# gau-nernst/centernet-lightning

Hardware: AMD Instinct MI355X
Metric: images/sec @512x512 ResNet34 CenterNet forward + gather_detection2d (higher is better)
Workload: dtype f32; 1 GPU; BASELINE C1: ResNet34 + simple neck, 32 img/GPU x 512x512, heads 80+4 (w256), k=100, nms 3; global_batch=32, per_gpu_batch=32, parallelism=batch-shard x1

## Files before the change

### centernet-lightning_amd/centernet_lightning_amd/_lib.py

```python
import ctypes
import os
from ctypes import (POINTER, Structure, c_char_p, c_double, c_float, c_int32, c_int64, c_size_t, c_uint32, c_void_p)

_LIB_NAME = "libcenternet_gfx950.so"
_LIB_PATH = os.path.join(os.path.dirname(os.path.abspath(__file__)), "lib", _LIB_NAME)

CNL_RELU = 1 << 0
CNL_SIGMOID = 1 << 1
CNL_UPSAMPLE_IN = 1 << 2
CNL_UPSAMPLE_OUT_ADD = 1 << 3
CNL_RELU6 = 1 << 4
CNL_W_SPLIT = 1 << 5

CNL_ALGO_AUTO, CNL_ALGO_F2, CNL_ALGO_F32, CNL_ALGO_LATENCY, CNL_ALGO_F43, CNL_ALGO_FORCE = 0, 1, 2, 4, 5, 100
CNL_WINO_F32, CNL_WINO_F16X2 = 2, 5

CNL_E_BAD_ARG, CNL_E_UNSUPPORTED, CNL_E_WORKSPACE, CNL_E_HIP = -1, -2, -3, -4
ABI_VERSION = 13


class ConvParams(Structure):
    _fields_ = [("x", c_void_p), ("w", c_void_p), ("bias", c_void_p), ("residual", c_void_p), ("y", c_void_p),
                ("N", c_int32), ("H_in", c_int32), ("W_in", c_int32), ("Cin", c_int32), ("Cout", c_int32),
                ("KH", c_int32), ("KW", c_int32), ("stride", c_int32), ("pad", c_int32),
                ("ldx", c_int32), ("ldy", c_int32), ("ldr", c_int32), ("flags", c_uint32),
                ("x_absmax", c_void_p), ("y_absmax", c_void_p), ("w_absmax", c_void_p), ("algo", c_uint32),
                ("splitk", c_int32), ("splitk_scratch", c_void_p), ("splitk_scratch_bytes", c_size_t),
                ("fuse_w", c_void_p), ("fuse_part", c_void_p), ("w_up", c_void_p)]


class DeconvParams(Structure):
    _fields_ = [("x", c_void_p), ("w", c_void_p), ("bias", c_void_p), ("residual", c_void_p), ("y", c_void_p),
                ("N", c_int32), ("H_in", c_int32), ("W_in", c_int32), ("Cin", c_int32), ("Cout", c_int32), ("K", c_int32),
                ("ldx", c_int32), ("ldy", c_int32), ("ldr", c_int32), ("flags", c_uint32)]

# ... 180 lines not shown
```

### centernet-lightning_amd/centernet_lightning_amd/engine.py

```python
import bisect
import ctypes
import threading
from collections import OrderedDict
from dataclasses import dataclass

import torch

from . import _lib
from ._lib import (CNL_ALGO_AUTO, CNL_ALGO_F2, CNL_ALGO_F32, CNL_ALGO_F43, CNL_ALGO_FORCE, CNL_ALGO_LATENCY, CNL_RELU, CNL_RELU6, CNL_SIGMOID, CNL_UPSAMPLE_IN, CNL_UPSAMPLE_OUT_ADD, CNL_W_SPLIT,
                   CNL_WINO_F16X2, ConvParams, DeconvParams)

BN_EPS_DEFAULT = 1e-5


@dataclass(frozen=True)
class KernelOptions:
    algo: str = "auto"
    winograd: bool = True
    up2: bool = True
    absmax_handover: bool = True
    stem_fused_pool: bool = True
    presplit_weights: bool = True
    fuse_small_out: bool = True
    reuse_buffers: bool = True
    split_small: bool = False
    latency: bool = False
    up_rows: bool = True
    f43: bool = False
    check_range: bool = False

    @property
    def algo_id(self):
        try:
            return {"auto": CNL_ALGO_AUTO, "f2": CNL_ALGO_F2, "f32": CNL_ALGO_F32}[self.algo]
        except KeyError:
            raise ValueError(f"KernelOptions.algo must be 'auto', 'f2' or 'f32', got {self.algo!r}") from None


def fold_conv_bn(conv_w, conv_b, bn=None):
    w = conv_w.detach().to(torch.float32)
    cout = w.shape[0]
    b = conv_b.detach().to(torch.float32) if conv_b is not None else torch.zeros(cout, device=w.device)
    if bn is not None:
        scale = bn.weight.detach().float() / torch.sqrt(bn.running_var.detach().float() + bn.eps)
        w = w * scale.view(-1, 1, 1, 1)
        b = (b - bn.running_mean.detach().float()) * scale + bn.bias.detach().float()
# ... 53 lines not shown
            stream = ctypes.c_void_p(torch.cuda.current_stream(self.w.device).cuda_stream)
            _lib.check(lib.cnl_up2_pack_weights_f32(self.w.data_ptr(), self._up2.data_ptr(), self.cin, self.cout, stream), "cnl_up2_pack_weights_f32")
            self.up2_wmax = self._up2.abs().max().reshape(1).contiguous()
    return self._up2


def _layer_up_rows(self):
    if getattr(self, "_up_rows", None) is None:
        lib = _lib.load()
        n = lib.cnl_winograd_up_weight_floats(self.cin, self.cout) if (self.w.is_cuda and self.kh == 3 and self.kw == 3 and self.stride == 1) else 0
        if not n:
            self._up_rows = False
        else:
            with torch.cuda.device(self.w.device):
                buf = torch.empty((n,), device=self.w.device, dtype=torch.float32)
                stream = ctypes.c_void_p(torch.cuda.current_stream(self.w.device).cuda_stream)
                _lib.check(lib.cnl_winograd_transform_weights_up_f32(self.w.data_ptr(), buf.data_ptr(), self.cin, self.cout, stream),
                           "cnl_winograd_transform_weights_up_f32")
                torch.cuda.current_stream(self.w.device).synchronize()
            self._up_rows = buf
    return self._up_rows if self._up_rows is not False else None


_Layer.up_rows = _layer_up_rows
_Layer.split_w = _layer_split_w
_Layer.wants_up2 = _layer_wants_up2
_Layer.up2 = _layer_up2


class _Bottleneck:

    def __init__(self, c1, c2, c3, down, li):
        self.c1, self.c2, self.c3, self.down, self.li = c1, c2, c3, down, li
        self.cat = None
        if down is not None:
            self.cat = _Layer(torch.cat([c3.w, down.w], dim=3).contiguous(), (c3.b + down.b).contiguous())
            self.cat.k1 = c3.cin


class _SepLayer:

    def __init__(self, mod, device):
        w = mod.dw.weight.detach().to(device=device, dtype=torch.float32)
        bn = mod.dw_bn
        scale = (bn.weight.detach().float() / torch.sqrt(bn.running_var.detach().float() + bn.eps)).to(device)
        self.dw_w = (w[:, 0] * scale.view(-1, 1, 1)).permute(1, 2, 0).contiguous()
        self.dw_b = (bn.bias.detach().float().to(device) - bn.running_mean.detach().float().to(device) * scale).contiguous()
# ... 499 lines not shown
            elif self.options.f43 and self.algo in (CNL_ALGO_AUTO, CNL_ALGO_F2):
                p.algo = CNL_ALGO_F43
        rowwino = (fn is self.lib.cnl_conv3x3_winograd_f32 and self.algo != CNL_ALGO_F32
                   and self.lib.cnl_conv3x3_winograd_variant(ctypes.byref(p)) in (9, 10, 11))
        if rowwino and self.options.up_rows and (flags & CNL_UPSAMPLE_IN) and residual is None:
            wu = layer.up_rows()
            if wu is not None:
                p.w_up = wu.data_ptr()
        if (self.options.up2 and (flags & CNL_UPSAMPLE_IN) and not (flags & ~(CNL_RELU | CNL_UPSAMPLE_IN)) and residual is None
                and layer.wants_up2() and not rowwino):
            p.w = layer.up2().data_ptr()
            p.w_absmax = layer.up2_wmax.data_ptr()
            p.algo = self.algo
            fn = self.lib.cnl_conv3x3_up2_nhwc_f32
            what = what.replace(" [winograd]", "") + " [sub-pixel phases]"
        if fn is self.lib.cnl_conv2d_nhwc_f32 and self.options.presplit_weights and self.algo != CNL_ALGO_F32:
            ws = layer.split_w()
            if ws is not None:
                p.w = ws.data_ptr()
                p.flags |= CNL_W_SPLIT
        self.launches.append(_Launch(fn, p, what, flops, keep=(x, y, residual, layer)))
        return p, ho.value, wo.value

    def _bottlenecks(self, Wt, cur, ch, cw, cc, feats):
        N = self.N
        pw_ok = self.algo in (CNL_ALGO_AUTO, CNL_ALGO_F2) and self.options.absmax_handover and _POINTWISE_AB != "generic_auto"
        for j, blk in enumerate(Wt.blocks):
            c1, c2, c3, down, li = blk.c1, blk.c2, blk.c3, blk.down, blk.li
            bi = j - next(i for i, b in enumerate(Wt.blocks) if b.li == li)
            name = f"layer{li + 1}.{bi}"
            t1 = self._buf(N, ch, cw, c1.cout)
            self._conv1x1(c1, cur, ch, cw, cc, t1, CNL_RELU, pw_ok, what=f"{name}.conv1")
            oh, ow = (ch + 2 - 3) // c2.stride + 1, (cw + 2 - 3) // c2.stride + 1
            t2 = self._buf(N, oh, ow, c2.cout)
            self._conv(c2, t1, ch, cw, c1.cout, t2, c2.cout, CNL_RELU, what=f"{name}.conv2")
            out = self._buf(N, oh, ow, c3.cout)
            if down is not None and pw_ok and _POINTWISE_AB in (None, "pointwise_all"):
                self._pointwise(blk.cat, t2, oh, ow, c2.cout, out, CNL_RELU, x2=(cur, ch, cw, cc, down.stride), what=f"{name}.conv3+downsample")
            else:
                idn = cur
                if down is not None:
                    idn = self._buf(N, oh, ow, down.cout)
                    self._conv1x1(down, cur, ch, cw, cc, idn, 0, pw_ok, what=f"{name}.downsample")
                self._conv1x1(c3, t2, oh, ow, c2.cout, out, CNL_RELU, pw_ok, residual=idn, what=f"{name}.conv3")
            cur, ch, cw, cc = out, oh, ow, c3.cout
            feats[li] = (cur, ch, cw, cc)
# ... 141 lines not shown
        self._wt_stem_packed = Wt.stem_packed
        if H % 32 or W % 32:
            raise ValueError(f"input H, W must be divisible by 32 (got {H}x{W}); docs/implementation.md:52 of the reference")
        h2, w2 = (H + 6 - 7) // 2 + 1, (W + 6 - 7) // 2 + 1
        h4, w4 = (h2 + 2 - 3) // 2 + 1, (w2 + 2 - 3) // 2 + 1
        cur = self._buf(N, h4, w4, 64)
        need_s1 = (Wt.neck_kind != "SimpleNeck" and len(Wt.fuse) >= 4) or not self.options.stem_fused_pool or self.algo == CNL_ALGO_F32
        s1 = self._buf(N, h2, w2, 64) if need_s1 else None
        self.stem_out = s1 if need_s1 else cur
        self.stem_fused_pool = not need_s1
        self.backbone_in = cur
        self.stem_absmax = None
        self.launches.append(_Launch("stem", None, "stem7x7+bn+relu" + ("" if need_s1 else "+maxpool3x3s2"), 2 * N * h2 * w2 * 64 * 147,
                                     keep=(self.stem_out,)))
        if need_s1:
            self.launches.append(_Launch("maxpool", (s1, cur, N, h2, w2, 64), "maxpool3x3s2", keep=(s1, cur)))
        ch, cw, cc = h4, w4, 64
        feats = {}
        if Wt.bottleneck:
            cur, ch, cw, cc = self._bottlenecks(Wt, cur, ch, cw, cc, feats)
        for bi, (c1, c2, down, li) in enumerate(() if Wt.bottleneck else Wt.blocks):
            oh, ow = (ch + 2 - 3) // c1.stride + 1, (cw + 2 - 3) // c1.stride + 1
            t = self._buf(N, oh, ow, c1.cout)
            self._conv(c1, cur, ch, cw, cc, t, c1.cout, CNL_RELU, what=f"layer{li + 1}.{bi}.conv1")
            if down is not None:
                idn = self._buf(N, oh, ow, down.cout)
                self._conv(down, cur, ch, cw, cc, idn, down.cout, 0, what=f"layer{li + 1}.{bi}.downsample")
            else:
                idn = cur
            out = self._buf(N, oh, ow, c2.cout)
            self._conv(c2, t, oh, ow, c1.cout, out, c2.cout, CNL_RELU, residual=idn, ldr=c2.cout, what=f"layer{li + 1}.{bi}.conv2")
            cur, ch, cw, cc = out, oh, ow, c2.cout
            feats[li] = (cur, ch, cw, cc)
        self.features = [(s1, h2, w2, 64)] + [feats[i] for i in range(4)]

        bil = 1 if Wt.upsample_type == "bilinear" else 0
        if Wt.neck_kind == "SimpleNeck":
            x, xh, xw, xc = self.features[-1]
            up = 0
            for i, (layer, dec) in enumerate(zip(Wt.neck_layers, Wt.neck_ups)):
                if up and isinstance(layer, (_SepLayer, _DeformLayer)):
                    x, xh, xw, up = self._upsample(x, xh, xw, xc, xc, 0, f"neck.upsample.{i - 1} (nearest)"), 2 * xh, 2 * xw, 0
                y = self._buf(N, xh * (2 if up else 1), xw * (2 if up else 1), layer.cout)
                oh, ow = self._block(layer, x, xh, xw, xc, y, layer.cout, f"neck.layers.{i}", up)
                x, xh, xw, xc, up = y, oh, ow, layer.cout, 0
                if dec is not None:
                    x, xh, xw = self._deconv(dec, x, xh, xw, xc, f"neck.upsamples.{i} (conv_transpose)"), 2 * xh, 2 * xw
                elif bil:
                    x, xh, xw = self._upsample(x, xh, xw, xc, xc, 1, f"neck.upsample.{i} (bilinear)"), 2 * xh, 2 * xw
                else:
                    up = CNL_UPSAMPLE_IN
# ... 337 lines not shown
```

### centernet-lightning_amd/csrc/conv_args.h

```cpp
#pragma once
#include "cnl_device.h"

namespace cnl_conv {
using namespace cnl_dev;


struct ConvArgs {
    const float* x;
    const float* w;
    const float* bias;
    const float* res;
    float* y;
    int N, Hin, Win, Cin, Cout;
    int KH, KW, stride, pad, pad_x;
    int sub_dy, sub_dx;
    int ldx, ldy, ldr;
    int HL, WL;
    int Ho, Wo, M;
    int CC, KT, K;
    unsigned x_bytes, w_bytes, y_bytes, r_bytes;
    unsigned flags;
    int tiles_n, tiles;
    unsigned mg_hw, sh_hw, mg_w, sh_w;
    long long* trace;
    const float* xmax;
    const float* wmax;
    unsigned* ymax;
    unsigned algo;
    const float* wscale;
    const float* wsplit = nullptr;
    int ksplit = 0, kt_per = 0;
    float* part = nullptr;
    unsigned part_bytes = 0;
};

constexpr unsigned CNL_I_SUBPIXEL = 1u << 16;

template <int WM, int WN, int TM, int TN>
struct Cfg {
    static constexpr int NW = WM * WN;
    static constexpr int THREADS = NW * 64;
    static constexpr int BM = WM * TM * 32;
    static constexpr int BN = WN * TN * 32;
    static constexpr int A_INSTR = BM / (NW * 8);
    static constexpr int B_INSTR = BN / (NW * 8);
    static constexpr int STAGE_BYTES = (BM + BN) * 128;
    static constexpr int LDS_BYTES = 2 * STAGE_BYTES;
    static_assert(NW == 4, "kernel is declared __launch_bounds__(256, 2)");
    static_assert(BM % (NW * 8) == 0 && BN % (NW * 8) == 0, "tile rows must split evenly over waves");
};


__device__ __forceinline__ f32x4 buf_load4(const float* base, unsigned bytes, unsigned voffset, unsigned soffset) {
    const auto rsrc = __builtin_amdgcn_make_buffer_rsrc((void*)base, 0, (int)bytes, 0x00020000);
    return __builtin_bit_cast(f32x4, __builtin_amdgcn_raw_buffer_load_b128(rsrc, voffset, soffset, 0));
}
// ... 16 lines not shown
```

### centernet-lightning_amd/csrc/conv_f16x2.hip

```cpp
#include "conv_args.h"
#include <cstdlib>

namespace cnl_conv {



template <int WM, int WN, int TM, int TN, int KS, bool SUB, bool SPLIT = false, bool PREB = false>
__global__ __launch_bounds__(256, 2) void conv_f16x2_kernel(const ConvArgs a) {
    using C = Cfg<WM, WN, TM, TN>;
    constexpr bool PRE = SUB || PREB;
    extern __shared__ __attribute__((aligned(16))) char smem[];
    float* sInv = reinterpret_cast<float*>(smem + C::LDS_BYTES);
    float* sScl = sInv + C::BM;
    int* sImg = reinterpret_cast<int*>(sScl + C::BM);
    unsigned* sPix = reinterpret_cast<unsigned*>(sImg + C::BM);

    const int lane = threadIdx.x & 63;
    const int wave = __builtin_amdgcn_readfirstlane(threadIdx.x >> 6);
    const int wm = wave / WN, wn = wave % WN;
    const int hi = lane >> 5;

    unsigned tile = cnl::xcd_remap(blockIdx.x, (unsigned)a.tiles);
    int slice = 0;
    if constexpr (SPLIT) { slice = (int)(tile % (unsigned)a.ksplit); tile /= (unsigned)a.ksplit; }
    const int kt0 = SPLIT ? slice * a.kt_per : 0;
    const int KTs = SPLIT ? min(a.kt_per, a.KT - kt0) : a.KT;
    const int n_tile = tile % a.tiles_n;
    const int m_tile = tile / a.tiles_n;
    const int m0 = m_tile * C::BM;
    const int n0 = n_tile * C::BN;

    const int lrow = lane >> 3;
    const int pslot = lane & 7;
    unsigned a_mask[C::A_INSTR], a_base[C::A_INSTR];
#pragma unroll
    for (int j = 0; j < C::A_INSTR; ++j) {
        const int r = (j * C::NW + wave) * 8 + lrow;
        const int m = m0 + r;
        const int q = (pslot ^ ((r >> 1) & 7)) * 4;
        const unsigned n = fast_div((unsigned)m, a.mg_hw, a.sh_hw);
        const unsigned rem = (unsigned)m - n * (unsigned)(a.Ho * a.Wo);
        const unsigned oy = fast_div(rem, a.mg_w, a.sh_w);
        const unsigned ox = rem - oy * (unsigned)a.Wo;
        const int iy0 = (int)oy * a.stride - a.pad;
        const int ix0 = (int)ox * a.stride - a.pad_x;
        unsigned mask = 0, xb = 0;
#pragma unroll
        for (int kx = 0; kx < KS; ++kx) xb |= ((unsigned)(ix0 + kx) < (unsigned)a.WL) ? (1u << kx) : 0u;
#pragma unroll
// ... 3 lines not shown
        a_base[j] = (unsigned)(((pix + iy0 * a.Win + ix0) * a.ldx + q) * 4);
    }
    unsigned b_off[C::B_INSTR];
#pragma unroll
    for (int j = 0; j < C::B_INSTR; ++j) {
        const int r = (j * C::NW + wave) * 8 + lrow;
        const int q = (pslot ^ ((r >> 1) & 7)) * 4;
        b_off[j] = (unsigned)(((n0 + r) * a.K + q) * 4);
    }
    unsigned a_voff[C::A_INSTR];
#define C5_TAP(tap_, ky_, kx_)                                                                                    \
    do {                                                                                                          \
        const unsigned bit_ = 1u << (tap_);                                                                       \
        const unsigned delta_ = (unsigned)((((ky_) * a.Win + (kx_)) * a.ldx) * 4);                                \
        _Pragma("unroll") for (int j = 0; j < C::A_INSTR; ++j) a_voff[j] = (a_mask[j] & bit_) ? a_base[j] + delta_ : OOB; \
    } while (0)
#define C5_ISSUE(stage_, c0_, kbase_)                                                                             \
    do {                                                                                                          \
        char* sA_ = smem + (stage_) * C::STAGE_BYTES;                                                             \
        char* sB_ = sA_ + C::BM * 128;                                                                            \
        _Pragma("unroll") for (int j = 0; j < C::A_INSTR; ++j)                                                    \
            dma16(a.x, a.x_bytes, sA_ + (j * C::NW + wave) * 1024, a_voff[j], (unsigned)((c0_) * 4));             \
        _Pragma("unroll") for (int j = 0; j < C::B_INSTR; ++j)                                                    \
            dma16(PREB ? a.wsplit : a.w, a.w_bytes, sB_ + (j * C::NW + wave) * 1024, b_off[j], (unsigned)((kbase_) * 4)); \
    } while (0)
    int tap = 0, ky = 0, kx = 0, cc = 0;
#define C5_ADVANCE()                                    \
    do {                                                \
        if (++cc == a.CC) {                             \
            cc = 0;                                     \
            ++tap;                                      \
            if (++kx == KS) { kx = 0; ++ky; }           \
            C5_TAP(tap, ky, kx);                        \
        }                                               \
    } while (0)
    if constexpr (SPLIT) {
        tap = kt0 / a.CC; cc = kt0 - tap * a.CC; ky = tap / KS; kx = tap - ky * KS;
    }
    C5_TAP(tap, ky, kx);
    C5_ISSUE(0, cc * 32, kt0 * 32);

    const float Sw = PRE ? *a.wscale : pow2_scale(*a.wmax);
    for (int r = threadIdx.x; r < C::BM; r += C::THREADS) {
        const int m = m0 + r;
        const unsigned n = fast_div((unsigned)m, a.mg_hw, a.sh_hw);
        const bool ok = m < a.M;
        const float S = ok ? pow2_scale(a.xmax[n * AMS]) : 1.f;
        sScl[r] = S;
        sInv[r] = 1.f / (S * Sw);
        sImg[r] = ok ? (int)n : -1;
        if constexpr (SUB) {
            const unsigned rem = (unsigned)m - n * (unsigned)(a.Ho * a.Wo);
            const unsigned oy = fast_div(rem, a.mg_w, a.sh_w);
            const unsigned ox = rem - oy * (unsigned)a.Wo;
            sPix[r] = (n * 2u * (unsigned)a.Ho + 2u * oy + (unsigned)a.sub_dy) * (2u * (unsigned)a.Wo) + 2u * ox + (unsigned)a.sub_dx;
        }
    }

    f32x16 acc[TM][TN];
#pragma unroll
    for (int i = 0; i < TM; ++i)
#pragma unroll
        for (int j = 0; j < TN; ++j) acc[i][j] = mfma_zero();

    const int swz = (lane >> 1) & 7;
// ... 68 lines not shown
#undef C5_READ
#undef C5_SPLIT
#undef C5_MFMA

    if constexpr (SPLIT) {
#pragma unroll
        for (int j = 0; j < TN; ++j) {
            const int col = n0 + (wn * TN + j) * 32 + (lane & 31);
#pragma unroll
            for (int i = 0; i < TM; ++i) {
                const int rl = (wm * TM + i) * 32 + 4 * hi;
                const int mb = m0 + rl;
#pragma unroll
                for (int r = 0; r < 16; ++r) {
                    const int ro = (r & 3) + 8 * (r >> 2);
                    const bool ok = col < a.Cout && mb + ro < a.M;
                    buf_store(acc[i][j][r] * sInv[rl + ro], a.part, a.part_bytes,
                              ok ? (unsigned)((((long long)slice * a.M + mb + ro) * a.Cout + col) * 4) : OOB, 0u);
                }
            }
        }
        return;
    }
    const float lo = (a.flags & (CNL_RELU | CNL_RELU6)) ? 0.f : -__builtin_inff();
    const float hi6 = (a.flags & CNL_RELU6) ? 6.f : __builtin_inff();
    const bool sigm = a.flags & CNL_SIGMOID;
    const int img0 = sImg[0];
    float omax = 0.f, omax1 = 0.f;
#pragma unroll
    for (int j = 0; j < TN; ++j) {
        const int col = n0 + (wn * TN + j) * 32 + (lane & 31);
        const bool col_ok = col < a.Cout;
        const float bv = col_ok ? a.bias[col] : 0.f;
#pragma unroll
        for (int i = 0; i < TM; ++i) {
            const int rl = (wm * TM + i) * 32 + 4 * hi;
            const int mb = m0 + rl;
            const unsigned y_voff = (unsigned)((mb * a.ldy + col) * 4);
            const unsigned r_voff = (unsigned)((mb * a.ldr + col) * 4);
            float v[16];
            bool ok[16];
#pragma unroll
            for (int r = 0; r < 16; ++r) {
                const int ro = (r & 3) + 8 * (r >> 2);
                ok[r] = col_ok && mb + ro < a.M;
                v[r] = acc[i][j][r] * sInv[rl + ro] + bv;
            }
            if (!SUB && a.res) {
                float rv[16];
#pragma unroll
                for (int r = 0; r < 16; ++r)
                    rv[r] = buf_load(a.res, a.r_bytes, ok[r] ? r_voff : OOB, (unsigned)(((r & 3) + 8 * (r >> 2)) * a.ldr * 4));
#pragma unroll
                for (int r = 0; r < 16; ++r) v[r] += rv[r];
            }
#pragma unroll
            for (int r = 0; r < 16; ++r) v[r] = fminf(fmaxf(v[r], lo), hi6);
            if (sigm) {
#pragma unroll
                for (int r = 0; r < 16; ++r) v[r] = cnl::fast_sigmoid(v[r]);
            }
            if constexpr (SUB) {
#pragma unroll
                for (int r = 0; r < 16; ++r)
                    buf_store(v[r], a.y, a.y_bytes, ok[r] ? (sPix[rl + (r & 3) + 8 * (r >> 2)] * (unsigned)a.ldy + (unsigned)col) * 4u : OOB, 0u);
            } else {
#pragma unroll
                for (int r = 0; r < 16; ++r)
                    buf_store(v[r], a.y, a.y_bytes, ok[r] ? y_voff : OOB, (unsigned)(((r & 3) + 8 * (r >> 2)) * a.ldy * 4));
            }
            if (a.ymax) {
#pragma unroll
                for (int r = 0; r < 16; ++r) {
                    const float av = ok[r] ? fabsf(v[r]) : 0.f;
                    const int img = sImg[rl + (r & 3) + 8 * (r >> 2)];
                    if (img == img0) omax = fmaxf(omax, av);
                    else if (img == img0 + 1) omax1 = fmaxf(omax1, av);
                    else if (av > 0.f) cnl::report_max(a.ymax + img * AMS, av);
                }
            }
        }
    }
    if (a.ymax) {
#pragma unroll
        for (int o = 32; o > 0; o >>= 1) {
            omax = fmaxf(omax, __shfl_xor(omax, o, 64));
            omax1 = fmaxf(omax1, __shfl_xor(omax1, o, 64));
        }
        if (lane == 0) cnl::report_max(a.ymax + img0 * AMS, omax);
        if (lane == 0) cnl::report_max(a.ymax + (img0 + 1) * AMS, omax1);
    }
}

__global__ __launch_bounds__(256) void splitk_reduce_kernel(const ConvArgs a) {
    const int C4 = (a.Cout + 3) / 4;
    const long total = (long)a.M * C4;
    const long t = (long)blockIdx.x * 256 + threadIdx.x;
    float omax = 0.f;
    int img = -1;
    if (t < total) {
        const int m = (int)(t / C4), col = (int)(t - (long)m * C4) * 4;
        img = (int)fast_div((unsigned)m, a.mg_hw, a.sh_hw);
        const bool vec = col + 4 <= a.Cout && (a.Cout & 3) == 0;
        float v[4] = {0.f, 0.f, 0.f, 0.f};
        const long sstride = (long)a.M * a.Cout;
        const float* p0 = a.part + (long)m * a.Cout + col;
        if (vec) {
            for (int s0 = 0; s0 < a.ksplit; s0 += 8) {
                f32x4 q[8];
#pragma unroll
                for (int j = 0; j < 8; ++j)
                    q[j] = s0 + j < a.ksplit ? *reinterpret_cast<const f32x4*>(p0 + (s0 + j) * sstride) : f32x4{0.f, 0.f, 0.f, 0.f};
#pragma unroll
// ... 31 lines not shown
            atomicMax(a.ymax + img * AMS, __float_as_uint(omax));
        }
    }
}

template <int KS>
static int launch_split5(const ConvArgs& in, hipStream_t stream) {
    using C = Cfg<2, 2, 1, 2>;
    ConvArgs a = in;
    const int tiles_m = (a.M + C::BM - 1) / C::BM;
    a.tiles_n = (a.Cout + C::BN - 1) / C::BN;
    a.tiles = tiles_m * a.tiles_n * a.ksplit;
    static cnl::DeviceOnce once;
    int rc = cnl::kernel_setup(once, reinterpret_cast<const void*>(&conv_f16x2_kernel<2, 2, 1, 2, KS, false, true>), 160 * 1024);
    if (rc != CNL_OK) return rc;
    hipLaunchKernelGGL((conv_f16x2_kernel<2, 2, 1, 2, KS, false, true>), dim3(a.tiles), dim3(C::THREADS), C::LDS_BYTES + C::BM * 16, stream, a);
    rc = cnl::check_launch("conv_f16x2_kernel (split)");
    if (rc != CNL_OK) return rc;
    const long total = (long)a.M * ((a.Cout + 3) / 4);
    hipLaunchKernelGGL(splitk_reduce_kernel, dim3((unsigned)((total + 255) / 256)), dim3(256), 0, stream, a);
    return cnl::check_launch("splitk_reduce_kernel");
}

template <int WM, int WN, int TM, int TN, int KS, bool SUB, bool PREB = false>
static int launch_one5(const ConvArgs& a, hipStream_t stream) {
    using C = Cfg<WM, WN, TM, TN>;
    static cnl::DeviceOnce once;
    const int rc = cnl::kernel_setup(once, reinterpret_cast<const void*>(&conv_f16x2_kernel<WM, WN, TM, TN, KS, SUB, false, PREB>), 160 * 1024);
    if (rc != CNL_OK) return rc;
    hipLaunchKernelGGL((conv_f16x2_kernel<WM, WN, TM, TN, KS, SUB, false, PREB>), dim3(a.tiles), dim3(C::THREADS), C::LDS_BYTES + C::BM * 16, stream, a);
    return cnl::check_launch("conv_f16x2_kernel");
}

template <int WM, int WN, int TM, int TN>
static int launch_cfg5(const ConvArgs& in, hipStream_t stream) {
    using C = Cfg<WM, WN, TM, TN>;
    ConvArgs a = in;
    const int tiles_m = (a.M + C::BM - 1) / C::BM;
    a.tiles_n = (a.Cout + C::BN - 1) / C::BN;
    a.tiles = tiles_m * a.tiles_n;
    if (a.flags & CNL_I_SUBPIXEL) return launch_one5<WM, WN, TM, TN, 2, true>(a, stream);
    if (a.wsplit) return a.KH == 3 ? launch_one5<WM, WN, TM, TN, 3, false, true>(a, stream) : launch_one5<WM, WN, TM, TN, 1, false, true>(a, stream);
    return a.KH == 3 ? launch_one5<WM, WN, TM, TN, 3, false>(a, stream) : launch_one5<WM, WN, TM, TN, 1, false>(a, stream);
}

bool f16x2_eligible(const ConvArgs& a) {
    const long long min_out_1x1 = a.algo == CNL_ALGO_FORCE + 5 ? 0 : (1ll << 20);
    if (a.algo == CNL_ALGO_F32 || !a.xmax || (a.flags & (CNL_UPSAMPLE_IN | CNL_UPSAMPLE_OUT_ADD))) return false;
    if (a.flags & CNL_I_SUBPIXEL) return a.KH == 2 && a.KW == 2 && !a.res && a.wscale;
    return (a.wmax || (a.wsplit && a.ksplit <= 1)) && a.KH == a.KW && (a.KH == 1 || a.KH == 3) && a.pad == a.pad_x &&
           (a.KH == 3 || a.ksplit > 1 || (long long)a.Ho * a.Wo * a.Cout >= min_out_1x1);
}

int f16x2_launch(const ConvArgs& a, hipStream_t s) {
    if (a.ksplit > 1 && !(a.flags & CNL_I_SUBPIXEL)) return a.KH == 3 ? launch_split5<3>(a, s) : launch_split5<1>(a, s);
    if (a.Cout <= 32) return launch_cfg5<4, 1, 2, 1>(a, s);
    if (a.Cout <= 64) return launch_cfg5<4, 1, 2, 2>(a, s);
    if (a.Cout <= 96) return launch_cfg5<4, 1, 1, 3>(a, s);
    const long long tiles128 = (((long long)a.M + 127) / 128) * ((a.Cout + 127) / 128);
    if (tiles128 < 512) return launch_cfg5<2, 2, 1, 2>(a, s);
    return launch_cfg5<4, 1, 1, 4>(a, s);
}

}
```

### centernet-lightning_amd/csrc/conv_mfma.hip

```cpp
#include "conv_args.h"
#include <cstdlib>

namespace cnl_conv {

__device__ __forceinline__ f32x16 mfma32(float a, float b, f32x16 c) {
    return __builtin_amdgcn_mfma_f32_32x32x2f32(a, b, c, 0, 0, 0);
}
__device__ __forceinline__ f32x16 mfma_zero() {
    const f32x16 z = {0.f, 0.f, 0.f, 0.f, 0.f, 0.f, 0.f, 0.f, 0.f, 0.f, 0.f, 0.f, 0.f, 0.f, 0.f, 0.f};
    return __builtin_amdgcn_mfma_f32_32x32x2f32(0.f, 0.f, z, 0, 0, 0);
}
template <bool CHECK, bool RES>
__device__ __forceinline__ void store_tile(const f32x16& acc, float bv, float lo, float hi6, bool sigm, const ConvArgs& a, unsigned y_voff,
                                           unsigned r_voff, int m_base, bool col_ok) {
    float v[16];
    if constexpr (RES) {
        float rv[16];
#pragma unroll
        for (int r = 0; r < 16; ++r) {
            const int ro = (r & 3) + 8 * (r >> 2);
            const bool ok = !CHECK || (col_ok && m_base + ro < a.M);
            rv[r] = buf_load(a.res, a.r_bytes, ok ? r_voff : OOB, (unsigned)(ro * a.ldr * 4));
        }
#pragma unroll
// ... 429 lines not shown
static int finish_and_launch(ConvArgs& a, bool out4x, const char* who, hipStream_t s) {
    CNL_REQUIRE(a.Ho > 0 && a.Wo > 0, CNL_E_BAD_ARG, "%s: empty output", who);
    const long long M = (long long)a.N * a.Ho * a.Wo;
    CNL_REQUIRE(M < (1ll << 31) - 512, CNL_E_UNSUPPORTED, "%s: N*Ho*Wo too large", who);
    a.M = (int)M;
    a.CC = a.Cin / 32; a.KT = a.KH * a.KW * a.CC; a.K = a.KH * a.KW * a.Cin;
    const unsigned long long lim = 0xFFFFFF00ull;
    const unsigned long long xb = (((unsigned long long)a.N * a.Hin * a.Win - 1) * a.ldx + a.Cin) * 4ull;
    const unsigned long long wb = (unsigned long long)a.Cout * a.K * 4ull;
    const unsigned long long Mo = out4x ? 4ull * M : (unsigned long long)M;
    const unsigned long long yb = ((Mo - 1) * a.ldy + a.Cout) * 4ull;
    const unsigned long long rb = a.res ? ((Mo - 1) * a.ldr + a.Cout) * 4ull : 0ull;
    CNL_REQUIRE(xb < lim && yb + 512ull * a.ldy * 4 < lim && rb + 512ull * a.ldr * 4 < lim, CNL_E_UNSUPPORTED,
                "%s: a tensor spans >= 4 GiB (x %llu, y %llu bytes); split the batch", who, xb, yb);
    CNL_REQUIRE(wb + (unsigned long long)256 * a.K * 4ull < lim, CNL_E_UNSUPPORTED, "%s: weight too large", who);
    a.x_bytes = (unsigned)xb; a.w_bytes = (unsigned)wb; a.y_bytes = (unsigned)yb; a.r_bytes = (unsigned)rb;
    a.tiles_n = a.tiles = 0;
    magic_u31((unsigned)(a.Ho * a.Wo), &a.mg_hw, &a.sh_hw);
    magic_u31((unsigned)a.Wo, &a.mg_w, &a.sh_w);
    a.trace = nullptr;
#ifdef CNL_TRACE
    if (const char* e = getenv("CNL_TRACE_PTR")) a.trace = (long long*)strtoull(e, nullptr, 0);
#endif
    if (f16x2_eligible(a)) {
        if (a.ksplit > 1) {
            const int per = (a.KT + a.ksplit - 1) / a.ksplit;
            const unsigned long long pb = (unsigned long long)a.ksplit * (unsigned long long)M * a.Cout * 4ull;
            if (per >= 2 && !out4x && !(a.flags & CNL_UPSAMPLE_IN) && pb < lim) {
                a.kt_per = per;
                a.ksplit = (a.KT + per - 1) / per;
                a.part_bytes = (unsigned)((unsigned long long)a.ksplit * (unsigned long long)M * a.Cout * 4ull);
            } else {
                a.ksplit = 0;
            }
        }
        return f16x2_launch(a, s);
    }
    a.ksplit = 0;
    if (a.Cout <= 32) return launch_cfg<4, 1, 2, 1>(a, s);
    if (a.Cout <= 64) return launch_cfg<4, 1, 2, 2>(a, s);
    if (a.Cout <= 96) return launch_cfg<4, 1, 1, 3>(a, s);
    const long long tiles128 = ((M + 127) / 128) * ((a.Cout + 127) / 128);
    if (tiles128 < 512) return launch_cfg<2, 2, 1, 2>(a, s);
    return launch_cfg<2, 2, 2, 2>(a, s);
}

// ... 39 lines not shown
                "cnl_conv2d_nhwc_f32: Cin=%d is not a multiple of 32 (use cnl_stem_conv7x7_f32 for the RGB stem)", p->Cin);
    CNL_REQUIRE(p->ldx >= p->Cin && p->ldy >= p->Cout && p->ldx % 4 == 0, CNL_E_BAD_ARG,
                "cnl_conv2d_nhwc_f32: pixel strides ldx=%d ldy=%d too small / misaligned", p->ldx, p->ldy);
    CNL_REQUIRE(((uintptr_t)p->x & 15) == 0 && ((uintptr_t)p->w & 15) == 0, CNL_E_BAD_ARG,
                "cnl_conv2d_nhwc_f32: x and w must be 16-byte aligned");
    const bool up_out = p->flags & CNL_UPSAMPLE_OUT_ADD;
    CNL_REQUIRE(!up_out || p->residual, CNL_E_BAD_ARG, "cnl_conv2d_nhwc_f32: CNL_UPSAMPLE_OUT_ADD needs a residual");
    CNL_REQUIRE(!up_out || !(p->flags & CNL_SIGMOID), CNL_E_UNSUPPORTED, "cnl_conv2d_nhwc_f32: sigmoid with UPSAMPLE_OUT_ADD");
    CNL_REQUIRE(!p->residual || p->ldr >= p->Cout, CNL_E_BAD_ARG, "cnl_conv2d_nhwc_f32: ldr=%d < Cout", p->ldr);

    ConvArgs a;
    a.x = p->x; a.w = p->w; a.bias = p->bias; a.res = p->residual; a.y = p->y;
    a.N = p->N; a.Hin = p->H_in; a.Win = p->W_in; a.Cin = p->Cin; a.Cout = p->Cout;
    a.KH = p->KH; a.KW = p->KW; a.stride = p->stride; a.pad = a.pad_x = p->pad;
    a.sub_dy = a.sub_dx = 0;
    a.ldx = p->ldx; a.ldy = p->ldy; a.ldr = p->ldr;
    a.flags = p->flags;
    a.xmax = p->x_absmax; a.wmax = p->w_absmax; a.ymax = reinterpret_cast<unsigned*>(p->y_absmax); a.wscale = nullptr; a.algo = p->algo;
    if (p->flags & CNL_W_SPLIT) {
        CNL_REQUIRE(p->KH == p->KW && (p->KH == 1 || p->KH == 3), CNL_E_BAD_ARG, "cnl_conv2d_nhwc_f32: CNL_W_SPLIT with a %d x %d kernel", p->KH, p->KW);
        const size_t total = (size_t)p->Cout * p->KH * p->KW * p->Cin;
        a.wsplit = p->w + total;
        a.wscale = p->w + 2 * total;
    }
    const int up = (p->flags & CNL_UPSAMPLE_IN) ? 2 : 1;
    a.HL = p->H_in * up; a.WL = p->W_in * up;
    a.Ho = (a.HL + 2 * p->pad - p->KH) / p->stride + 1;
    a.Wo = (a.WL + 2 * p->pad - p->KW) / p->stride + 1;
    if (p->splitk > 1) {
        CNL_REQUIRE(p->splitk <= 256, CNL_E_BAD_ARG, "cnl_conv2d_nhwc_f32: splitk=%d (at most 256 slices)", p->splitk);
        CNL_REQUIRE(p->splitk_scratch && ((uintptr_t)p->splitk_scratch & 15) == 0 && p->splitk_scratch_bytes >= cnl_conv2d_splitk_scratch_bytes(p),
                    CNL_E_WORKSPACE, "cnl_conv2d_nhwc_f32: splitk_scratch missing, unaligned or smaller than cnl_conv2d_splitk_scratch_bytes()");
        a.ksplit = p->splitk;
        a.part = p->splitk_scratch;
    }
    return finish_and_launch(a, up_out, "cnl_conv2d_nhwc_f32", (hipStream_t)stream);
}

namespace cnl_conv {
__global__ __launch_bounds__(256) void up2_pack_kernel(const float* __restrict__ w, float* __restrict__ wp, int Cin, int Cout) {
    const long total = 16l * Cin * Cout;
    for (long e = (long)blockIdx.x * 256 + threadIdx.x; e < total; e += (long)gridDim.x * 256) {
        const int ci = (int)(e % Cin);
        long t = e / Cin;
        const int kx2 = (int)(t & 1), ky2 = (int)((t >> 1) & 1);
        t >>= 2;
// ... 189 lines not shown
```

### include/centernet_gfx950.h

```cpp
#ifndef CENTERNET_GFX950_H
#define CENTERNET_GFX950_H

#include <stddef.h>
#include <stdint.h>

#ifdef __cplusplus
extern "C" {
#endif
#if defined(__GNUC__) || defined(__clang__)
#pragma GCC visibility push(default)
#endif

#define CNL_ABI_VERSION 13

enum {
    CNL_OK = 0,
    CNL_E_BAD_ARG = -1,
    CNL_E_UNSUPPORTED = -2,
    CNL_E_WORKSPACE = -3,
    CNL_E_HIP = -4
};

enum {
    CNL_ALGO_AUTO = 0,
    CNL_ALGO_F2 = 1,
    CNL_ALGO_F32 = 2,
    CNL_ALGO_LATENCY = 4,
    CNL_ALGO_F43 = 5,
    CNL_ALGO_FORCE = 100
};

enum {
    CNL_RELU = 1u << 0,
    CNL_SIGMOID = 1u << 1,
    CNL_UPSAMPLE_IN = 1u << 2,
    CNL_UPSAMPLE_OUT_ADD = 1u << 3,
    CNL_RELU6 = 1u << 4,
    CNL_W_SPLIT = 1u << 5
};

typedef struct cnl_conv_params {
    const float* x;
    const float* w;
    const float* bias;
    const float* residual;
    float* y;
    int32_t N, H_in, W_in, Cin, Cout;
    int32_t KH, KW, stride, pad;
    int32_t ldx, ldy, ldr;
    uint32_t flags;
    const float* x_absmax;
    float* y_absmax;
    const float* w_absmax;
    uint32_t algo;
    int32_t splitk;
    float* splitk_scratch;
    size_t splitk_scratch_bytes;
    const float* fuse_w;
    float* fuse_part;
    const float* w_up;
} cnl_conv_params;
// ... 177 lines not shown
```

Measured before the change: 4262 images/s.

## Fuse 1x1 stride-2 downsample into the first 3x3 conv of basic blocks

Adds a CNL_FUSE_DOWNSAMPLE path that lets the stride-2 3x3 conv1 kernel run a second pass in the same workgroup. That pass computes the 1x1 stride-2 downsample from the same input tile, reusing the centre-tap addressing, and writes the identity branch with its own bias and scale. This removes a separate kernel launch and its input reads for each transition block in the ResNet34 layers 2 to 4. The cost is a longer kernel per tile and a second load of the input channels, and it only applies when the fp16-split path without split-K is chosen.

```diff
diff --git a/centernet-lightning_amd/centernet_lightning_amd/_lib.py b/centernet-lightning_amd/centernet_lightning_amd/_lib.py
--- a/centernet-lightning_amd/centernet_lightning_amd/_lib.py
+++ b/centernet-lightning_amd/centernet_lightning_amd/_lib.py
@@ -11,6 +11,7 @@
 CNL_UPSAMPLE_OUT_ADD = 1 << 3
 CNL_RELU6 = 1 << 4
 CNL_W_SPLIT = 1 << 5
+CNL_FUSE_DOWNSAMPLE = 1 << 6
 
 CNL_ALGO_AUTO, CNL_ALGO_F2, CNL_ALGO_F32, CNL_ALGO_LATENCY, CNL_ALGO_F43, CNL_ALGO_FORCE = 0, 1, 2, 4, 5, 100
 CNL_WINO_F32, CNL_WINO_F16X2 = 2, 5
diff --git a/centernet-lightning_amd/centernet_lightning_amd/engine.py b/centernet-lightning_amd/centernet_lightning_amd/engine.py
--- a/centernet-lightning_amd/centernet_lightning_amd/engine.py
+++ b/centernet-lightning_amd/centernet_lightning_amd/engine.py
@@ -7,7 +7,7 @@
 import torch
 
 from . import _lib
-from ._lib import (CNL_ALGO_AUTO, CNL_ALGO_F2, CNL_ALGO_F32, CNL_ALGO_F43, CNL_ALGO_FORCE, CNL_ALGO_LATENCY, CNL_RELU, CNL_RELU6, CNL_SIGMOID, CNL_UPSAMPLE_IN, CNL_UPSAMPLE_OUT_ADD, CNL_W_SPLIT,
+from ._lib import (CNL_ALGO_AUTO, CNL_ALGO_F2, CNL_ALGO_F32, CNL_ALGO_F43, CNL_ALGO_FORCE, CNL_ALGO_LATENCY, CNL_RELU, CNL_RELU6, CNL_SIGMOID, CNL_UPSAMPLE_IN, CNL_UPSAMPLE_OUT_ADD, CNL_W_SPLIT, CNL_FUSE_DOWNSAMPLE,
                    CNL_WINO_F16X2, ConvParams, DeconvParams)
 
 BN_EPS_DEFAULT = 1e-5
@@ -22,6 +22,7 @@
     stem_fused_pool: bool = True
     presplit_weights: bool = True
     fuse_small_out: bool = True
+    fuse_downsample: bool = True
     reuse_buffers: bool = True
     split_small: bool = False
     latency: bool = False
@@ -121,7 +122,22 @@
     return self._up_rows if self._up_rows is not False else None
 
 
+def _layer_ds_w(self):
+    if getattr(self, "_ds_w", None) is None:
+        lib = _lib.load()
+        n = lib.cnl_conv_split_weight_floats(self.cin, self.cout, 1, 1)
+        with torch.cuda.device(self.w.device):
+            buf = torch.empty((n + self.cout,), device=self.w.device, dtype=torch.float32)
+            stream = ctypes.c_void_p(torch.cuda.current_stream(self.w.device).cuda_stream)
+            _lib.check(lib.cnl_conv_split_weights_f32(self.w.data_ptr(), buf.data_ptr(), self.cin, self.cout, 1, 1, stream), "cnl_conv_split_weights_f32")
+            buf[n:].copy_(self.b)
+            torch.cuda.current_stream(self.w.device).synchronize()
+        self._ds_w = buf
+    return self._ds_w
+
+
 _Layer.up_rows = _layer_up_rows
+_Layer.ds_w = _layer_ds_w
 _Layer.split_w = _layer_split_w
 _Layer.wants_up2 = _layer_wants_up2
 _Layer.up2 = _layer_up2
@@ -667,6 +683,23 @@
         self.launches.append(_Launch(fn, p, what, flops, keep=(x, y, residual, layer)))
         return p, ho.value, wo.value
 
+    def _fuses_downsample(self, c1, down, oh, ow):
+        o = self.options
+        return (o.fuse_downsample and self.algo in (CNL_ALGO_AUTO, CNL_ALGO_F2) and o.absmax_handover and o.presplit_weights
+                and (c1.kh, c1.kw, c1.stride, c1.pad) == (3, 3, 2, 1) and (down.kh, down.kw, down.stride) == (1, 1, 2)
+                and c1.cout == down.cout and c1.cout > 96 and c1.cin == down.cin and c1.cin % 32 == 0 and c1.w.is_cuda
+                and self._split_slices(c1, CNL_RELU, oh, ow) <= 1)
+
+    def _conv_downsample(self, c1, down, x, xh, xw, ldx, y, idn, what):
+        p, oh, ow = self._conv(c1, x, xh, xw, ldx, y, c1.cout, CNL_RELU, what=what)
+        L = self.launches[-1]
+        assert L.args is p and L.fn is self.lib.cnl_conv2d_nhwc_f32 and (p.flags & CNL_W_SPLIT), what
+        p.flags |= CNL_FUSE_DOWNSAMPLE
+        p.w_up = down.ds_w().data_ptr()
+        p.fuse_part = idn.data_ptr()
+        L.flops += 2 * self.N * oh * ow * down.cout * down.cin
+        L.keep = L.keep + (idn, down)
+
     def _bottlenecks(self, Wt, cur, ch, cw, cc, feats):
         N = self.N
         pw_ok = self.algo in (CNL_ALGO_AUTO, CNL_ALGO_F2) and self.options.absmax_handover and _POINTWISE_AB != "generic_auto"
@@ -854,11 +887,15 @@
         for bi, (c1, c2, down, li) in enumerate(() if Wt.bottleneck else Wt.blocks):
             oh, ow = (ch + 2 - 3) // c1.stride + 1, (cw + 2 - 3) // c1.stride + 1
             t = self._buf(N, oh, ow, c1.cout)
-            self._conv(c1, cur, ch, cw, cc, t, c1.cout, CNL_RELU, what=f"layer{li + 1}.{bi}.conv1")
-            if down is not None:
+            if down is not None and self._fuses_downsample(c1, down, oh, ow):
+                idn = self._buf(N, oh, ow, down.cout)
+                self._conv_downsample(c1, down, cur, ch, cw, cc, t, idn, what=f"layer{li + 1}.{bi}.conv1+downsample")
+            elif down is not None:
+                self._conv(c1, cur, ch, cw, cc, t, c1.cout, CNL_RELU, what=f"layer{li + 1}.{bi}.conv1")
                 idn = self._buf(N, oh, ow, down.cout)
                 self._conv(down, cur, ch, cw, cc, idn, down.cout, 0, what=f"layer{li + 1}.{bi}.downsample")
             else:
+                self._conv(c1, cur, ch, cw, cc, t, c1.cout, CNL_RELU, what=f"layer{li + 1}.{bi}.conv1")
                 idn = cur
             out = self._buf(N, oh, ow, c2.cout)
             self._conv(c2, t, oh, ow, c1.cout, out, c2.cout, CNL_RELU, residual=idn, ldr=c2.cout, what=f"layer{li + 1}.{bi}.conv2")
diff --git a/centernet-lightning_amd/csrc/conv_args.h b/centernet-lightning_amd/csrc/conv_args.h
--- a/centernet-lightning_amd/csrc/conv_args.h
+++ b/centernet-lightning_amd/csrc/conv_args.h
@@ -32,6 +32,11 @@
     int ksplit = 0, kt_per = 0;
     float* part = nullptr;
     unsigned part_bytes = 0;
+    const float* ds_wsplit = nullptr;
+    const float* ds_wscale = nullptr;
+    const float* ds_bias = nullptr;
+    float* ds_y = nullptr;
+    unsigned ds_w_bytes = 0, ds_y_bytes = 0;
 };
 
 constexpr unsigned CNL_I_SUBPIXEL = 1u << 16;
diff --git a/centernet-lightning_amd/csrc/conv_f16x2.hip b/centernet-lightning_amd/csrc/conv_f16x2.hip
--- a/centernet-lightning_amd/csrc/conv_f16x2.hip
+++ b/centernet-lightning_amd/csrc/conv_f16x2.hip
@@ -5,10 +5,11 @@
 
 
 
-template <int WM, int WN, int TM, int TN, int KS, bool SUB, bool SPLIT = false, bool PREB = false>
+template <int WM, int WN, int TM, int TN, int KS, bool SUB, bool SPLIT = false, bool PREB = false, bool DS = false>
 __global__ __launch_bounds__(256, 2) void conv_f16x2_kernel(const ConvArgs a) {
     using C = Cfg<WM, WN, TM, TN>;
     constexpr bool PRE = SUB || PREB;
+    static_assert(!DS || (KS == 3 && PREB && !SUB && !SPLIT), "the fused downsample rides on the pre-split 3x3 form");
     extern __shared__ __attribute__((aligned(16))) char smem[];
     float* sInv = reinterpret_cast<float*>(smem + C::LDS_BYTES);
     float* sScl = sInv + C::BM;
@@ -24,7 +25,7 @@
     int slice = 0;
     if constexpr (SPLIT) { slice = (int)(tile % (unsigned)a.ksplit); tile /= (unsigned)a.ksplit; }
     const int kt0 = SPLIT ? slice * a.kt_per : 0;
-    const int KTs = SPLIT ? min(a.kt_per, a.KT - kt0) : a.KT;
+    int KTs = SPLIT ? min(a.kt_per, a.KT - kt0) : a.KT;
     const int n_tile = tile % a.tiles_n;
     const int m_tile = tile / a.tiles_n;
     const int m0 = m_tile * C::BM;
@@ -74,9 +75,24 @@
         _Pragma("unroll") for (int j = 0; j < C::A_INSTR; ++j)                                                    \
             dma16(a.x, a.x_bytes, sA_ + (j * C::NW + wave) * 1024, a_voff[j], (unsigned)((c0_) * 4));             \
         _Pragma("unroll") for (int j = 0; j < C::B_INSTR; ++j)                                                    \
-            dma16(PREB ? a.wsplit : a.w, a.w_bytes, sB_ + (j * C::NW + wave) * 1024, b_off[j], (unsigned)((kbase_) * 4)); \
-    } while (0)
+            dma16(p2 ? a.ds_wsplit : (PREB ? a.wsplit : a.w), p2 ? a.ds_w_bytes : a.w_bytes, sB_ + (j * C::NW + wave) * 1024, b_off[j], (unsigned)((kbase_) * 4)); \
+    } while (0)
+    bool p2 = false;
+second_pass:
     int tap = 0, ky = 0, kx = 0, cc = 0;
+    if constexpr (DS) {
+        if (p2) {
+            __syncthreads();
+            KTs = a.CC;
+            tap = 4; ky = 1; kx = 1;
+#pragma unroll
+            for (int j = 0; j < C::B_INSTR; ++j) {
+                const int r = (j * C::NW + wave) * 8 + lrow;
+                const int q = (pslot ^ ((r >> 1) & 7)) * 4;
+                b_off[j] = (unsigned)(((n0 + r) * a.Cin + q) * 4);
+            }
+        }
+    }
 #define C5_ADVANCE()                                    \
     do {                                                \
         if (++cc == a.CC) {                             \
@@ -92,7 +108,7 @@
     C5_TAP(tap, ky, kx);
     C5_ISSUE(0, cc * 32, kt0 * 32);
 
-    const float Sw = PRE ? *a.wscale : pow2_scale(*a.wmax);
+    const float Sw = p2 ? *a.ds_wscale : (PRE ? *a.wscale : pow2_scale(*a.wmax));
     for (int r = threadIdx.x; r < C::BM; r += C::THREADS) {
         const int m = m0 + r;
         const unsigned n = fast_div((unsigned)m, a.mg_hw, a.sh_hw);
@@ -207,21 +223,28 @@
         }
         return;
     }
-    const float lo = (a.flags & (CNL_RELU | CNL_RELU6)) ? 0.f : -__builtin_inff();
-    const float hi6 = (a.flags & CNL_RELU6) ? 6.f : __builtin_inff();
-    const bool sigm = a.flags & CNL_SIGMOID;
+    const unsigned eflags = p2 ? 0u : a.flags;
+    const float* ebias = p2 ? a.ds_bias : a.bias;
+    const float* eres = p2 ? nullptr : a.res;
+    float* ey = p2 ? a.ds_y : a.y;
+    const unsigned ey_bytes = p2 ? a.ds_y_bytes : a.y_bytes;
+    const int eldy = p2 ? a.Cout : a.ldy;
+    unsigned* eymax = p2 ? nullptr : a.ymax;
+    const float lo = (eflags & (CNL_RELU | CNL_RELU6)) ? 0.f : -__builtin_inff();
+    const float hi6 = (eflags & CNL_RELU6) ? 6.f : __builtin_inff();
+    const bool sigm = eflags & CNL_SIGMOID;
     const int img0 = sImg[0];
     float omax = 0.f, omax1 = 0.f;
 #pragma unroll
     for (int j = 0; j < TN; ++j) {
         const int col = n0 + (wn * TN + j) * 32 + (lane & 31);
         const bool col_ok = col < a.Cout;
-        const float bv = col_ok ? a.bias[col] : 0.f;
+        const float bv = col_ok ? ebias[col] : 0.f;
 #pragma unroll
         for (int i = 0; i < TM; ++i) {
             const int rl = (wm * TM + i) * 32 + 4 * hi;
             const int mb = m0 + rl;
-            const unsigned y_voff = (unsigned)((mb * a.ldy + col) * 4);
+            const unsigned y_voff = (unsigned)((mb * eldy + col) * 4);
             const unsigned r_voff = (unsigned)((mb * a.ldr + col) * 4);
             float v[16];
             bool ok[16];
@@ -231,11 +254,11 @@
                 ok[r] = col_ok && mb + ro < a.M;
                 v[r] = acc[i][j][r] * sInv[rl + ro] + bv;
             }
-            if (!SUB && a.res) {
+            if (!SUB && eres) {
                 float rv[16];
 #pragma unroll
                 for (int r = 0; r < 16; ++r)
-                    rv[r] = buf_load(a.res, a.r_bytes, ok[r] ? r_voff : OOB, (unsigned)(((r & 3) + 8 * (r >> 2)) * a.ldr * 4));
+                    rv[r] = buf_load(eres, a.r_bytes, ok[r] ? r_voff : OOB, (unsigned)(((r & 3) + 8 * (r >> 2)) * a.ldr * 4));
 #pragma unroll
                 for (int r = 0; r < 16; ++r) v[r] += rv[r];
             }
@@ -248,32 +271,38 @@
             if constexpr (SUB) {
 #pragma unroll
                 for (int r = 0; r < 16; ++r)
-                    buf_store(v[r], a.y, a.y_bytes, ok[r] ? (sPix[rl + (r & 3) + 8 * (r >> 2)] * (unsigned)a.ldy + (unsigned)col) * 4u : OOB, 0u);
+                    buf_store(v[r], ey, ey_bytes, ok[r] ? (sPix[rl + (r & 3) + 8 * (r >> 2)] * (unsigned)eldy + (unsigned)col) * 4u : OOB, 0u);
             } else {
 #pragma unroll
                 for (int r = 0; r < 16; ++r)
-                    buf_store(v[r], a.y, a.y_bytes, ok[r] ? y_voff : OOB, (unsigned)(((r & 3) + 8 * (r >> 2)) * a.ldy * 4));
-            }
-            if (a.ymax) {
+                    buf_store(v[r], ey, ey_bytes, ok[r] ? y_voff : OOB, (unsigned)(((r & 3) + 8 * (r >> 2)) * eldy * 4));
+            }
+            if (eymax) {
 #pragma unroll
                 for (int r = 0; r < 16; ++r) {
                     const float av = ok[r] ? fabsf(v[r]) : 0.f;
                     const int img = sImg[rl + (r & 3) + 8 * (r >> 2)];
                     if (img == img0) omax = fmaxf(omax, av);
                     else if (img == img0 + 1) omax1 = fmaxf(omax1, av);
-                    else if (av > 0.f) cnl::report_max(a.ymax + img * AMS, av);
+                    else if (av > 0.f) cnl::report_max(eymax + img * AMS, av);
                 }
             }
         }
     }
-    if (a.ymax) {
+    if (eymax) {
 #pragma unroll
         for (int o = 32; o > 0; o >>= 1) {
             omax = fmaxf(omax, __shfl_xor(omax, o, 64));
             omax1 = fmaxf(omax1, __shfl_xor(omax1, o, 64));
         }
-        if (lane == 0) cnl::report_max(a.ymax + img0 * AMS, omax);
-        if (lane == 0) cnl::report_max(a.ymax + (img0 + 1) * AMS, omax1);
+        if (lane == 0) cnl::report_max(eymax + img0 * AMS, omax);
+        if (lane == 0) cnl::report_max(eymax + (img0 + 1) * AMS, omax1);
+    }
+    if constexpr (DS) {
+        if (!p2) {
+            p2 = true;
+            goto second_pass;
+        }
     }
 }
 
@@ -351,23 +380,24 @@
     return cnl::check_launch("splitk_reduce_kernel");
 }
 
-template <int WM, int WN, int TM, int TN, int KS, bool SUB, bool PREB = false>
+template <int WM, int WN, int TM, int TN, int KS, bool SUB, bool PREB = false, bool DS = false>
 static int launch_one5(const ConvArgs& a, hipStream_t stream) {
     using C = Cfg<WM, WN, TM, TN>;
     static cnl::DeviceOnce once;
-    const int rc = cnl::kernel_setup(once, reinterpret_cast<const void*>(&conv_f16x2_kernel<WM, WN, TM, TN, KS, SUB, false, PREB>), 160 * 1024);
+    const int rc = cnl::kernel_setup(once, reinterpret_cast<const void*>(&conv_f16x2_kernel<WM, WN, TM, TN, KS, SUB, false, PREB, DS>), 160 * 1024);
     if (rc != CNL_OK) return rc;
-    hipLaunchKernelGGL((conv_f16x2_kernel<WM, WN, TM, TN, KS, SUB, false, PREB>), dim3(a.tiles), dim3(C::THREADS), C::LDS_BYTES + C::BM * 16, stream, a);
+    hipLaunchKernelGGL((conv_f16x2_kernel<WM, WN, TM, TN, KS, SUB, false, PREB, DS>), dim3(a.tiles), dim3(C::THREADS), C::LDS_BYTES + C::BM * 16, stream, a);
     return cnl::check_launch("conv_f16x2_kernel");
 }
 
-template <int WM, int WN, int TM, int TN>
+template <int WM, int WN, int TM, int TN, bool DS = false>
 static int launch_cfg5(const ConvArgs& in, hipStream_t stream) {
     using C = Cfg<WM, WN, TM, TN>;
     ConvArgs a = in;
     const int tiles_m = (a.M + C::BM - 1) / C::BM;
     a.tiles_n = (a.Cout + C::BN - 1) / C::BN;
     a.tiles = tiles_m * a.tiles_n;
+    if constexpr (DS) return launch_one5<WM, WN, TM, TN, 3, false, true, true>(a, stream);
     if (a.flags & CNL_I_SUBPIXEL) return launch_one5<WM, WN, TM, TN, 2, true>(a, stream);
     if (a.wsplit) return a.KH == 3 ? launch_one5<WM, WN, TM, TN, 3, false, true>(a, stream) : launch_one5<WM, WN, TM, TN, 1, false, true>(a, stream);
     return a.KH == 3 ? launch_one5<WM, WN, TM, TN, 3, false>(a, stream) : launch_one5<WM, WN, TM, TN, 1, false>(a, stream);
@@ -387,6 +417,7 @@
     if (a.Cout <= 64) return launch_cfg5<4, 1, 2, 2>(a, s);
     if (a.Cout <= 96) return launch_cfg5<4, 1, 1, 3>(a, s);
     const long long tiles128 = (((long long)a.M + 127) / 128) * ((a.Cout + 127) / 128);
+    if (a.ds_y) return tiles128 < 512 ? launch_cfg5<2, 2, 1, 2, true>(a, s) : launch_cfg5<4, 1, 1, 4, true>(a, s);
     if (tiles128 < 512) return launch_cfg5<2, 2, 1, 2>(a, s);
     return launch_cfg5<4, 1, 1, 4>(a, s);
 }
diff --git a/centernet-lightning_amd/csrc/conv_mfma.hip b/centernet-lightning_amd/csrc/conv_mfma.hip
--- a/centernet-lightning_amd/csrc/conv_mfma.hip
+++ b/centernet-lightning_amd/csrc/conv_mfma.hip
@@ -475,6 +475,15 @@
 #ifdef CNL_TRACE
     if (const char* e = getenv("CNL_TRACE_PTR")) a.trace = (long long*)strtoull(e, nullptr, 0);
 #endif
+    if (a.ds_y) {
+        CNL_REQUIRE(a.KH == 3 && a.KW == 3 && a.stride == 2 && a.pad == 1 && a.wsplit && a.ksplit <= 1 && !out4x && !(a.flags & CNL_UPSAMPLE_IN) && a.Cout > 96 &&
+                        f16x2_eligible(a), CNL_E_UNSUPPORTED,
+                    "%s: CNL_FUSE_DOWNSAMPLE needs a 3x3 / stride 2 / pad 1 conv on the fp16-split kernel (x_absmax, CNL_W_SPLIT, Cout > 96, algo AUTO / F2, no splitk, no upsampling)", who);
+        const unsigned long long dyb = (unsigned long long)M * a.Cout * 4ull;
+        CNL_REQUIRE(dyb + 512ull * a.Cout * 4 < lim, CNL_E_UNSUPPORTED, "%s: the downsample output spans >= 4 GiB; split the batch", who);
+        a.ds_w_bytes = (unsigned)((unsigned long long)a.Cout * a.Cin * 4ull);
+        a.ds_y_bytes = (unsigned)dyb;
+    }
     if (f16x2_eligible(a)) {
         if (a.ksplit > 1) {
             const int per = (a.KT + a.ksplit - 1) / a.ksplit;
@@ -560,6 +569,15 @@
         const size_t total = (size_t)p->Cout * p->KH * p->KW * p->Cin;
         a.wsplit = p->w + total;
         a.wscale = p->w + 2 * total;
+    }
+    if ((p->flags & CNL_FUSE_DOWNSAMPLE) && p->w_up) {
+        CNL_REQUIRE(p->fuse_part && !p->fuse_w, CNL_E_BAD_ARG, "cnl_conv2d_nhwc_f32: CNL_FUSE_DOWNSAMPLE needs fuse_part (the downsample's output) and no fuse_w");
+        CNL_REQUIRE(((uintptr_t)p->w_up & 15) == 0, CNL_E_BAD_ARG, "cnl_conv2d_nhwc_f32: the downsample weights (w_up) must be 16-byte aligned");
+        const size_t total1 = (size_t)p->Cout * p->Cin;
+        a.ds_wsplit = p->w_up + total1;
+        a.ds_wscale = p->w_up + 2 * total1;
+        a.ds_bias = p->w_up + cnl_conv_split_weight_floats(p->Cin, p->Cout, 1, 1);
+        a.ds_y = p->fuse_part;
     }
     const int up = (p->flags & CNL_UPSAMPLE_IN) ? 2 : 1;
     a.HL = p->H_in * up; a.WL = p->W_in * up;
diff --git a/include/centernet_gfx950.h b/include/centernet_gfx950.h
--- a/include/centernet_gfx950.h
+++ b/include/centernet_gfx950.h
@@ -36,7 +36,8 @@
     CNL_UPSAMPLE_IN = 1u << 2,
     CNL_UPSAMPLE_OUT_ADD = 1u << 3,
     CNL_RELU6 = 1u << 4,
-    CNL_W_SPLIT = 1u << 5
+    CNL_W_SPLIT = 1u << 5,
+    CNL_FUSE_DOWNSAMPLE = 1u << 6
 };
 
 typedef struct cnl_conv_params {
```

Result: no change. 4293 images/s (median of 6 runs) (+0.7%).
